# muzishen/RCDMs

Hardware: AMD Instinct MI355X
Metric: story-frames/sec (stage-2 UNet, 50-step DDIM, 512^2) (higher is better)
Workload: dtype f16; 1 GPU; PororoSV stage-2, 512x512, 50-step DDIM, CFG 2.0, batch=1 story x 5 frames per GPU, ctx 85x768, random-init 1276.9M-param UNet3D; stories_per_gpu=1, latent=64, ddim_steps=50, parallelism=story-replicas x1

## Files before the change

### rcdms_amd/csrc/igemm16.hip

```cpp
#include "common.h"
#include "igemm_args.h"
#include "pp_sync.h"
#include "igemm_epilogue.h"
#ifndef RCDM_I16_ABLATE
#define RCDM_I16_ABLATE 0
#endif

namespace {

template <int TAPS, bool SLAB>
__global__ __launch_bounds__(256, 2) void igemm16_kernel(const IgemmArgs p) {
  constexpr int BM = 160, BN = 160, FM = 5, FN = 5;
  constexpr int A_BYTES = BM * 128, STAGE = (BM + BN) * 128;
  constexpr int NP = BM / 8 / 4;
  extern __shared__ __attribute__((aligned(16))) char smem[];

  const int t = threadIdx.x, lane = t & 63;
  const int wave = __builtin_amdgcn_readfirstlane(t >> 6);
  const int wm = wave >> 1, wn = wave & 1;
  const int ks_begin = blockIdx.y * p.nk_per_split;
  const int nkl = min(p.nk, ks_begin + p.nk_per_split) - ks_begin;
  if (nkl <= 0) return;

  int cm0, cn0;
  {
    const int ntiles = p.tilesM * p.tilesN, lin = blockIdx.x;
    const int xcd = lin & 7, q = ntiles >> 3, r = ntiles & 7;
    const int tl = (xcd < r ? xcd * (q + 1) : r * (q + 1) + (xcd - r) * q) + (lin >> 3);
    constexpr int GM = 8;
    const int per_group = GM * p.tilesN;
    const int sg = tl / per_group, rem = tl - sg * per_group;
    const int gm = min(GM, p.tilesM - sg * GM);
    const int tn = rem / gm, tm = sg * GM + (rem - tn * gm);
    cm0 = tm * BM;
    cn0 = tn * BN;
  }

  f32x2 lx_pre = {1.f, 0.f};
  const bool lx_on = TAPS == 1 && !SLAB && p.lnx_stat != nullptr;
  LnxRow<1, kLnxMaxParts> lx_row0;
  if (lx_on && t < BM) lx_row0.load(p.lnx_stat, p.lnx_ld, cm0 + t, cm0 + t < p.M, p.lnx_parts, 0);

  const __amdgpu_buffer_rsrc_t rsrcA = __builtin_amdgcn_make_buffer_rsrc((void*)p.A, 0, 0x7FFFFFFF, 0x00020000);
  const __amdgpu_buffer_rsrc_t rsrcW = __builtin_amdgcn_make_buffer_rsrc((void*)p.W, 0, 0x7FFFFFFF, 0x00020000);
  const __amdgpu_buffer_rsrc_t rsrcA2 = __builtin_amdgcn_make_buffer_rsrc((void*)(TAPS == 9 ? p.A2 : p.A), 0, 0x7FFFFFFF, 0x00020000);
  constexpr unsigned OOB = 0x80000000u;
  const int Hv = p.Hi << p.up, Wv = p.Wi << p.up;
  const int lrow = lane >> 3, lch = lane & 7;

  unsigned a_off[NP], w_off[NP];
  int a_img[NP], a_iy[NP], a_ix[NP], a_c[NP], w_c[NP];
#pragma unroll
  for (int i = 0; i < NP; ++i) {
    const int row = (wave * NP + i) * 8 + lrow;
    const int m = cm0 + row;
    a_c[i] = (lch ^ ((row >> 1) & 7)) * 8;
    a_off[i] = OOB;
    a_img[i] = a_ix[i] = 0;
    a_iy[i] = -(1 << 20);
    if (TAPS == 1) {
      if (m < p.M) a_off[i] = (unsigned)m * (unsigned)p.lda * 2u;
    } else if (m < p.M) {
      const int hw = p.Ho * p.Wo;
      const int img = m / hw, rem = m - img * hw;
      const int oy = rem / p.Wo, ox = rem - oy * p.Wo;
      a_img[i] = img * p.Hi * p.Wi;
      a_iy[i] = oy * p.stride - p.pad;
      a_ix[i] = ox * p.stride - p.pad;
    }
    const int n = cn0 + row;
    w_c[i] = a_c[i];
    w_off[i] = n < p.N ? (unsigned)n * (unsigned)p.Ktot * 2u : OOB;
  }
  auto issue = [&](int g, int stage) __attribute__((always_inline)) {
    const int ks = ks_begin + g;
    int tap = 0, kci = ks;
    const bool s2 = TAPS == 9 && ks >= p.nk1;
    if (TAPS != 1) {
      kci = ks / 9;
      tap = ks - kci * 9;
      if (s2) {
        kci = ks - p.nk1;
        tap = 9;
      }
    }
    const int c0 = kci * BK;
    const int dy = s2 ? 1 : tap / 3, dx = s2 ? 1 : tap - dy * 3;
    const int cin = s2 ? p.Cin2 : p.Cin;
    const unsigned lda = (unsigned)(s2 ? p.lda2 : p.lda);
    char* sbase = smem + stage * STAGE;
#pragma unroll
    for (int i = 0; i < NP; ++i) {
      const int c = c0 + a_c[i];
      unsigned vo;
      if (TAPS == 1) {
        vo = (c < p.Cin && a_off[i] != OOB) ? a_off[i] + (unsigned)c * 2u : OOB;
      } else {
        const int iy = a_iy[i] + dy, ix = a_ix[i] + dx;
        const bool ok = (c < cin) && ((unsigned)iy < (unsigned)Hv) && ((unsigned)ix < (unsigned)Wv);
        const int sy = iy >> p.up, sx = ix >> p.up;
        const unsigned off = ((unsigned)(a_img[i] + sy * p.Wi + sx) * lda + (unsigned)c) * 2u;
        vo = ok ? off : OOB;
      }
      if (TAPS == 9 && s2)
        __builtin_amdgcn_raw_ptr_buffer_load_lds(
            rsrcA2, (__attribute__((address_space(3))) void*)(sbase + (wave * NP + i) * 1024), 16, vo, 0, 0, 0);
      else
        __builtin_amdgcn_raw_ptr_buffer_load_lds(
            rsrcA, (__attribute__((address_space(3))) void*)(sbase + (wave * NP + i) * 1024), 16, vo, 0, 0, 0);
    }
#if RCDM_I16_ABLATE & 16
    if (g > 0) return;
#endif
#pragma unroll
    for (int i = 0; i < NP; ++i) {
      const int c = c0 + w_c[i];
      const unsigned vo = (c < cin && w_off[i] != OOB)
                              ? w_off[i] + ((unsigned)tap * (unsigned)p.Cin + (unsigned)c) * 2u : OOB;
      __builtin_amdgcn_raw_ptr_buffer_load_lds(
          rsrcW, (__attribute__((address_space(3))) void*)(sbase + A_BYTES + (wave * NP + i) * 1024), 16, vo, 0, 0, 0);
    }
  };

  const int l15 = lane & 15, kg = lane >> 4;
  const int sw = (lane >> 1) & 7;
  const int koff0 = ((kg ^ sw) << 4), koff1 = (((4 + kg) ^ sw) << 4);
  const int rowA = (wm * (BM / 2) + l15) * 128, rowB = A_BYTES + (wn * (BN / 2) + l15) * 128;
  f32x4 acc[FN][FM];
#pragma unroll
  for (int i = 0; i < FN; ++i)
#pragma unroll
    for (int j = 0; j < FM; ++j) acc[i][j] = f32x4{0.f, 0.f, 0.f, 0.f};

  constexpr int kStg = BM * (2 * BN + 16);
  static_assert(lnx_table_bytes(BM, BN) <= 4096 && 4096 + kStg <= 2 * STAGE && kStg >= STAGE, "epilogue layout");
  const bool lx_low = lx_on && !(nkl & 1);
  float* const lx_tab = (float*)(smem + (lx_low ? 0 : kStg));
  char* const stg = smem + (lx_low ? 4096 : 0);
  issue(0, 0);
  if (lx_on && t < BM) {
    float r_ = 1.f, m_ = 0.f;
    lx_row0.finish(p.lnx_invC, p.lnx_eps, r_, m_);
    lx_pre = f32x2{r_, m_};
  }
  for (int g = 0; g < nkl; ++g) {
    wait_vm<0>();
    __builtin_amdgcn_s_barrier();
#if !(RCDM_I16_ABLATE & 8)
    if (g + 1 < nkl) issue(g + 1, (g + 1) & 1);
#endif
    const char* sb = smem + (g & 1) * STAGE;
#if RCDM_PRIO_LOADS
    __builtin_amdgcn_s_setprio(3);
#endif
#pragma unroll
    for (int kk = 0; kk < 2; ++kk) {
      const int koff = kk ? koff1 : koff0;
      f16x8 wf[FN], xf[FM];
#pragma unroll
      for (int i = 0; i < FN; ++i) wf[i] = *(const f16x8*)(sb + rowB + i * 2048 + koff);
#pragma unroll
      for (int j = 0; j < FM; ++j) xf[j] = *(const f16x8*)(sb + rowA + j * 2048 + koff);
#if RCDM_PRIO_LOADS
      __builtin_amdgcn_s_setprio(0);
#endif
#pragma unroll
      for (int i = 0; i < FN; ++i)
#pragma unroll
        for (int j = 0; j < FM; ++j) acc[i][j] = __builtin_amdgcn_mfma_f32_16x16x32_f16(wf[i], xf[j], acc[i][j], 0, 0, 0);
#if RCDM_PRIO_LOADS
      __builtin_amdgcn_s_setprio(3);
#endif
    }
  }
  if constexpr (TAPS == 1 && !SLAB)
    if (lx_on) lnx_write_tables<BM, BN>(p, lx_tab, cm0, cn0, t, lx_pre);
  wait_lgkm0();
  tick_barrier();
#if RCDM_I16_ABLATE & 1
  {
    float s = 0.f;
#pragma unroll
    for (int i = 0; i < FN; ++i)
#pragma unroll
      for (int j = 0; j < FM; ++j) s += acc[i][j][0] + acc[i][j][1] + acc[i][j][2] + acc[i][j][3];
    if (s == 1.2345678e33f) p.out[0] = (f16)s;
  }
#else
  if constexpr (SLAB) {
    if (p.slab16) {
      IgemmArgs q{};
      q.out = (f16*)p.partial + (size_t)blockIdx.y * p.M * p.N;
      q.M = p.M; q.N = p.N; q.ldc = p.N; q.epi = 0; q.out_scale = 1.0f; q.dup = 0;
      tile_epilogue<FM, FN, false, 256, BM, BN, false, false>(q, smem, acc, cm0, cn0, wm * (BM / 2), wn * (BN / 2), l15, kg, t, nullptr);
      return;
    }
  }
  tile_epilogue<FM, FN, SLAB, 256, BM, BN, false, TAPS == 1 && !SLAB>(p, stg, acc, cm0, cn0, wm * (BM / 2), wn * (BN / 2), l15, kg, t,
                                                                       lx_on ? lx_tab : nullptr);
#endif
}

constexpr int kLds16 = 2 * (160 + 160) * 128;

template <int TAPS>
int launch16(const IgemmArgs& a, hipStream_t stream) {
  static bool attr_set[64] = {};
  if (rcdm_first_on_device(attr_set)) {
    (void)hipFuncSetAttribute((const void*)igemm16_kernel<TAPS, false>, hipFuncAttributeMaxDynamicSharedMemorySize, kLds16);
    (void)hipFuncSetAttribute((const void*)igemm16_kernel<TAPS, true>, hipFuncAttributeMaxDynamicSharedMemorySize, kLds16);
  }
  dim3 grid(a.tilesM * a.tilesN, a.splits);
  if (a.splits > 1)
    hipLaunchKernelGGL((igemm16_kernel<TAPS, true>), grid, dim3(256), kLds16, stream, a);
  else
    hipLaunchKernelGGL((igemm16_kernel<TAPS, false>), grid, dim3(256), kLds16, stream, a);
  return rcdm_check_launch();
}

}

int rcdm_igemm16_launch(const IgemmArgs& a, int taps, hipStream_t stream) {
  if (taps == 1) return launch16<1>(a, stream);
  if (taps == 9) return launch16<9>(a, stream);
  return RCDM_EINVAL;
}
```

### rcdms_amd/csrc/wino.hip

```cpp
#include "common.h"
#include "igemm_args.h"
#include "pp_sync.h"
#include "igemm_epilogue.h"
#include <stdlib.h>

namespace {

struct WinoArgs {
  const f16* in;
  const f16* in2;
  const f16* U;
  const f16* W2;
  const float* bias;
  const float* rowvec;
  const f16* res;
  f16* out;
  f16* V;
  float* slab;
  int slab16;
  int n_img, H, W, th, tw, T, N, K, K2;
  int lda, lda2, ldc, ldr, ldt, rows_per_sample;
  int epi;
  float out_scale;
  int E, splits, nk, nk2, nkps, nkps2, tilesM, tilesN;
  const float* gn_stat;
  const float* gn_gamma;
  const float* gn_beta;
  int gn_cg, gn_G, gn_rps, gn_silu;
  float* go_partial;
  int go_G, go_cg, go_rps, go_splits;
};

__global__ __launch_bounds__(256) void wino_in_kernel(const WinoArgs p) {
  const int nch = p.K >> 2;
  const int idx = blockIdx.x * 256 + threadIdx.x;
  if (idx >= p.T * nch) return;
  const int t = idx / nch, c4 = idx - t * nch;
  const int tpi = p.th * p.tw;
  const int img = t / tpi, rem = t - img * tpi;
  const int ty = rem / p.tw, tx = rem - ty * p.tw;
  typedef unsigned u32x2_t __attribute__((ext_vector_type(2)));
  union H4 { u32x2_t v; f16 e[4]; f16x4 h; };
  const __amdgpu_buffer_rsrc_t rs = __builtin_amdgcn_make_buffer_rsrc((void*)p.in, 0, 0x7FFFFFFF, 0x00020000);
  const unsigned base = ((unsigned)(img * p.H * p.W) * (unsigned)p.lda + (unsigned)c4 * 4u) * 2u;
  H4 d[4][4];
  bool ok[4][4];
#pragma unroll
  for (int i = 0; i < 4; ++i)
#pragma unroll
    for (int j = 0; j < 4; ++j) {
      const int y = 2 * ty - 1 + i, x = 2 * tx - 1 + j;
      ok[i][j] = (unsigned)y < (unsigned)p.H && (unsigned)x < (unsigned)p.W;
      const unsigned off = ok[i][j] ? base + (unsigned)(y * p.W + x) * (unsigned)p.lda * 2u : 0x80000000u;
      d[i][j].v = __builtin_amdgcn_raw_buffer_load_b64(rs, off, 0, 0);
    }
  f32x4 sc = {1.f, 1.f, 1.f, 1.f}, sh = {0.f, 0.f, 0.f, 0.f};
  const bool gn = p.gn_stat != nullptr;
  if (gn) {
    const int s = (img * p.H * p.W) / p.gn_rps;
    const f32x4 ga = *(const f32x4*)(p.gn_gamma + c4 * 4), be = *(const f32x4*)(p.gn_beta + c4 * 4);
#pragma unroll
    for (int e = 0; e < 4; ++e) {
      const int g = (c4 * 4 + e) / p.gn_cg;
      const f32x2 mr = *(const f32x2*)(p.gn_stat + (size_t)(s * p.gn_G + g) * 2);
      sc[e] = mr.y * ga[e];
      sh[e] = __builtin_fmaf(-(mr.x * mr.y), ga[e], be[e]);
    }
  }
  float f[4][4][4];
#pragma unroll
  for (int i = 0; i < 4; ++i)
#pragma unroll
    for (int j = 0; j < 4; ++j)
#pragma unroll
      for (int e = 0; e < 4; ++e) {
        float v = (float)d[i][j].e[e];
        if (gn) {
          v = __builtin_fmaf(v, sc[e], sh[e]);
          if (p.gn_silu) v = silu_f(v);
          if (!ok[i][j]) v = 0.f;
        }
        f[i][j][e] = v;
      }
  float r[4][4][4];
#pragma unroll
  for (int j = 0; j < 4; ++j)
#pragma unroll
    for (int e = 0; e < 4; ++e) {
      r[0][j][e] = f[0][j][e] - f[2][j][e];
      r[1][j][e] = f[1][j][e] + f[2][j][e];
      r[2][j][e] = f[2][j][e] - f[1][j][e];
      r[3][j][e] = f[1][j][e] - f[3][j][e];
    }
  f16* vb = p.V + (size_t)t * p.K + c4 * 4;
  const size_t pstride = (size_t)p.T * p.K;
#pragma unroll
  for (int i = 0; i < 4; ++i) {
    H4 o[4];
#pragma unroll
    for (int e = 0; e < 4; ++e) {
      o[0].e[e] = (f16)(r[i][0][e] - r[i][2][e]);
      o[1].e[e] = (f16)(r[i][1][e] + r[i][2][e]);
      o[2].e[e] = (f16)(r[i][2][e] - r[i][1][e]);
      o[3].e[e] = (f16)(r[i][1][e] - r[i][3][e]);
    }
#pragma unroll
    for (int j = 0; j < 4; ++j) *(u32x2_t*)(vb + (size_t)(i * 4 + j) * pstride) = o[j].v;
  }
}

template <bool S16>
__global__ __launch_bounds__(256, 2) void wino_gemm_kernel(const WinoArgs p) {
  constexpr int BM = 160, BN = 160, FM = 5, FN = 5;
  constexpr int A_BYTES = BM * 128, STAGE = (BM + BN) * 128;
  constexpr int NP = BM / 8 / 4;
  extern __shared__ __attribute__((aligned(16))) char smem[];

  const int t = threadIdx.x, lane = t & 63;
  const int wave = __builtin_amdgcn_readfirstlane(t >> 6);
  const int wm = wave >> 1, wn = wave & 1;
  const int ntile = p.tilesM * p.tilesN, W = p.E * p.splits * ntile;
  const int n_extra = p.E - 16;
  int item;
  {
    const int lin = blockIdx.x, xcd = lin & 7, j = lin >> 3;
    const int WX = n_extra * p.splits * ntile, WM = W - WX;
    if (((WX | WM) & 7) == 0) {
      const int xq = WX >> 3, mq = WM >> 3;
      item = j < xq ? xcd * xq + j : WX + xcd * mq + (j - xq);
    } else {
      const int q = W >> 3, r = W & 7;
      item = (xcd < r ? xcd * (q + 1) : r * (q + 1) + (xcd - r) * q) + j;
    }
  }
  const int yes = item / ntile, tl = item - yes * ntile;
  const int ye = yes / p.splits, split = yes - ye * p.splits;
  const int entry = ye < n_extra ? 16 + ye : ye - n_extra;
  const bool extra = entry >= 16;
  const int nk = extra ? p.nk2 : p.nk, nkps = extra ? p.nkps2 : p.nkps;
  const int ks_begin = split * nkps;
  const int nkl = min(nk, ks_begin + nkps) - ks_begin;
  const int Kd = extra ? p.K2 : p.K;
  const size_t slab_off = ((size_t)entry * p.splits + split) * p.T * p.N;

  const int tn = tl / p.tilesM, tm = tl - tn * p.tilesM;
  const int cm0 = tm * BM, cn0 = tn * BN;
  const f16* Abase = extra ? p.in2 : p.V + (size_t)entry * p.T * p.K;
  const f16* Wbase = extra ? p.W2 : p.U + (size_t)entry * p.N * p.K;
  const __amdgpu_buffer_rsrc_t rsrcA = __builtin_amdgcn_make_buffer_rsrc((void*)Abase, 0, 0x7FFFFFFF, 0x00020000);
  const __amdgpu_buffer_rsrc_t rsrcW = __builtin_amdgcn_make_buffer_rsrc((void*)Wbase, 0, 0x7FFFFFFF, 0x00020000);
  constexpr unsigned OOB = 0x80000000u;
  const int lrow = lane >> 3, lch = lane & 7;

  unsigned a_off[NP], w_off[NP];
  int a_c[NP];
#pragma unroll
  for (int i = 0; i < NP; ++i) {
    const int row = (wave * NP + i) * 8 + lrow;
    const int m = cm0 + row;
    a_c[i] = (lch ^ ((row >> 1) & 7)) * 8;
    a_off[i] = OOB;
    if (m < p.T) {
      if (extra) {
        const int tpi = p.th * p.tw;
        const int img = m / tpi, rem = m - img * tpi;
        const int ty = rem / p.tw, tx = rem - ty * p.tw;
        const int ab = entry - 16;
        const int prow = img * p.H * p.W + (2 * ty + (ab >> 1)) * p.W + 2 * tx + (ab & 1);
        a_off[i] = (unsigned)prow * (unsigned)p.lda2 * 2u;
      } else {
        a_off[i] = (unsigned)m * (unsigned)p.K * 2u;
      }
    }
    const int n = cn0 + row;
    w_off[i] = n < p.N ? (unsigned)n * (unsigned)Kd * 2u : OOB;
  }
  auto issue = [&](int g, int stage) __attribute__((always_inline)) {
    const int c0 = (ks_begin + g) * BK;
    char* sbase = smem + stage * STAGE;
#pragma unroll
    for (int i = 0; i < NP; ++i) {
      const int c = c0 + a_c[i];
      const unsigned vo = (c < Kd && a_off[i] != OOB) ? a_off[i] + (unsigned)c * 2u : OOB;
      __builtin_amdgcn_raw_ptr_buffer_load_lds(
          rsrcA, (__attribute__((address_space(3))) void*)(sbase + (wave * NP + i) * 1024), 16, vo, 0, 0, 0);
    }
#pragma unroll
    for (int i = 0; i < NP; ++i) {
      const int c = c0 + a_c[i];
      const unsigned vo = (c < Kd && w_off[i] != OOB) ? w_off[i] + (unsigned)c * 2u : OOB;
      __builtin_amdgcn_raw_ptr_buffer_load_lds(
          rsrcW, (__attribute__((address_space(3))) void*)(sbase + A_BYTES + (wave * NP + i) * 1024), 16, vo, 0, 0, 0);
    }
  };

  const int l15 = lane & 15, kg = lane >> 4;
  const int sw = (lane >> 1) & 7;
  const int koff0 = ((kg ^ sw) << 4), koff1 = (((4 + kg) ^ sw) << 4);
  const int rowA = (wm * (BM / 2) + l15) * 128, rowB = A_BYTES + (wn * (BN / 2) + l15) * 128;
  f32x4 acc[FN][FM];
#pragma unroll
  for (int i = 0; i < FN; ++i)
#pragma unroll
    for (int j = 0; j < FM; ++j) acc[i][j] = f32x4{0.f, 0.f, 0.f, 0.f};

  if (nkl > 0) issue(0, 0);
  for (int g = 0; g < nkl; ++g) {
    wait_vm<0>();
    __builtin_amdgcn_s_barrier();
    if (g + 1 < nkl) issue(g + 1, (g + 1) & 1);
    const char* sb = smem + (g & 1) * STAGE;
    __builtin_amdgcn_s_setprio(3);
#pragma unroll
    for (int kk = 0; kk < 2; ++kk) {
      const int koff = kk ? koff1 : koff0;
      f16x8 wf[FN], xf[FM];
#pragma unroll
      for (int i = 0; i < FN; ++i) wf[i] = *(const f16x8*)(sb + rowB + i * 2048 + koff);
#pragma unroll
      for (int j = 0; j < FM; ++j) xf[j] = *(const f16x8*)(sb + rowA + j * 2048 + koff);
      __builtin_amdgcn_s_setprio(0);
#pragma unroll
      for (int i = 0; i < FN; ++i)
#pragma unroll
        for (int j = 0; j < FM; ++j) acc[i][j] = __builtin_amdgcn_mfma_f32_16x16x32_f16(wf[i], xf[j], acc[i][j], 0, 0, 0);
      __builtin_amdgcn_s_setprio(3);
    }
  }
  const int row0 = wm * (BM / 2), col0 = wn * (BN / 2);
  if constexpr (S16) {
    wait_lgkm0();
    tick_barrier();
    IgemmArgs q{};
    q.out = (f16*)p.slab + slab_off;
    q.M = p.T; q.N = p.N; q.ldc = p.N; q.epi = 0; q.out_scale = 1.0f; q.dup = 0;
    tile_epilogue<FM, FN, false, 256, BM, BN, false, false>(q, smem, acc, cm0, cn0, row0, col0, l15, kg, t, nullptr);
  } else {
    wait_lgkm0();
    tick_barrier();
    slab_store_staged<FM, FN, 256, BM, BN, 80>(p.slab + slab_off, p.N, p.T, p.N, smem, acc, cm0, cn0, row0, col0, l15, kg, t);
  }
}

template <bool S16>
__device__ __forceinline__ f32x4 slab_load4(const WinoArgs& p, size_t off) {
  if constexpr (S16) {
    union { uint2 u; f16 e[4]; } h;
    h.u = *(const uint2*)((const f16*)p.slab + off);
    return f32x4{(float)h.e[0], (float)h.e[1], (float)h.e[2], (float)h.e[3]};
  } else {
    return *(const f32x4*)(p.slab + off);
  }
}

template <int SP, bool S16>
__global__ __launch_bounds__(512) void wino_out_kernel(const WinoArgs p) {
  extern __shared__ __attribute__((aligned(16))) char smem[];
  const int nch = p.N >> 2;
  const int t = blockIdx.x;
  const int tpi = p.th * p.tw;
  const int img = t / tpi, rem = t - img * tpi;
  const int ty = rem / p.tw, tx = rem - ty * p.tw;
  const size_t splane = (size_t)p.T * p.N, eplane = (size_t)p.splits * splane;
  int prow[4];
#pragma unroll
  for (int ab = 0; ab < 4; ++ab) prow[ab] = img * p.H * p.W + (2 * ty + (ab >> 1)) * p.W + 2 * tx + (ab & 1);
  union H4 { uint2 u; f16 e[4]; };
  for (int cg4 = threadIdx.x; cg4 < nch; cg4 += blockDim.x) {
    const int n = cg4 * 4;
    const size_t src = (size_t)t * p.N + n;
    H4 rr[4];
#pragma unroll
    for (int ab = 0; ab < 4; ++ab) {
      rr[ab].u = make_uint2(0, 0);
      if (p.epi & RCDM_EPI_RESIDUAL) rr[ab].u = *(const uint2*)(p.res + (size_t)prow[ab] * p.ldr + n);
    }
    f32x4 m[16];
#pragma unroll
    for (int e = 0; e < 16; ++e) m[e] = slab_load4<S16>(p, src + e * eplane);
    if constexpr (SP == 2) {
      f32x4 m2[16];
#pragma unroll
      for (int e = 0; e < 16; ++e) m2[e] = slab_load4<S16>(p, src + e * eplane + splane);
#pragma unroll
      for (int e = 0; e < 16; ++e) m[e] += m2[e];
    } else if constexpr (SP == 0) {
      for (int s = 1; s < p.splits; ++s) {
        f32x4 m2[16];
#pragma unroll
        for (int e = 0; e < 16; ++e) m2[e] = slab_load4<S16>(p, src + e * eplane + s * splane);
#pragma unroll
        for (int e = 0; e < 16; ++e) m[e] += m2[e];
      }
    }
    f32x4 o[4];
    {
      f32x4 r0[4], r1[4];
#pragma unroll
      for (int j = 0; j < 4; ++j) {
        r0[j] = m[0 * 4 + j] + m[1 * 4 + j] + m[2 * 4 + j];
        r1[j] = m[1 * 4 + j] - m[2 * 4 + j] - m[3 * 4 + j];
      }
      o[0] = r0[0] + r0[1] + r0[2];
      o[1] = r0[1] - r0[2] - r0[3];
      o[2] = r1[0] + r1[1] + r1[2];
      o[3] = r1[1] - r1[2] - r1[3];
    }
    if (p.E > 16) {
      f32x4 x[4];
#pragma unroll
      for (int ab = 0; ab < 4; ++ab) x[ab] = slab_load4<S16>(p, src + (16 + ab) * eplane);
      for (int s = 1; s < p.splits; ++s) {
#pragma unroll
        for (int ab = 0; ab < 4; ++ab) x[ab] += slab_load4<S16>(p, src + (16 + ab) * eplane + s * splane);
      }
#pragma unroll
      for (int ab = 0; ab < 4; ++ab) o[ab] += x[ab];
    }
    f32x4 add = {0.f, 0.f, 0.f, 0.f};
    if (p.epi & RCDM_EPI_BIAS) add += *(const f32x4*)(p.bias + n);
    if (p.epi & RCDM_EPI_ROWVEC) add += *(const f32x4*)(p.rowvec + (size_t)(prow[0] / p.rows_per_sample) * p.ldt + n);
    f32x4 cs = {0.f, 0.f, 0.f, 0.f}, cq = cs;
#pragma unroll
    for (int ab = 0; ab < 4; ++ab) {
      H4 q;
#pragma unroll
      for (int e = 0; e < 4; ++e) {
        q.e[e] = (f16)((o[ab][e] + add[e] + (float)rr[ab].e[e]) * p.out_scale);
        const float f = (float)q.e[e];
        cs[e] += f;
        cq[e] += f * f;
      }
      *(uint2*)(p.out + (size_t)prow[ab] * p.ldc + n) = q.u;
    }
    if (p.go_partial) {
      *(f32x4*)(smem + (size_t)n * 4) = cs;
      *(f32x4*)(smem + (size_t)(p.N + n) * 4) = cq;
    }
  }
  if (p.go_partial) {
    __syncthreads();
    const int g = threadIdx.x;
    if (g < p.go_G) {
      const float* fs = (const float*)smem;
      float gs = 0.f, gq = 0.f;
      for (int c = g * p.go_cg; c < (g + 1) * p.go_cg; ++c) {
        gs += fs[c];
        gq += fs[p.N + c];
      }
      const float nn = 4.f * (float)p.go_cg;
      const float mean = gs / nn;
      float m2 = gq - gs * mean;
      if (m2 < 0.f) m2 = 0.f;
      const int s = prow[0] / p.go_rps;
      const int sp = t - s * p.go_splits;
      float* o = p.go_partial + (((size_t)s * p.go_G + g) * p.go_splits + sp) * 3;
      o[0] = nn;
      o[1] = mean;
      o[2] = m2;
    }
  }
}

__global__ __launch_bounds__(256) void wino_pack_kernel(const float* __restrict__ w, f16* __restrict__ U, int c_out, int c_in) {
  const size_t idx = (size_t)blockIdx.x * 256 + threadIdx.x;
  const size_t total = (size_t)c_out * c_in;
  if (idx >= total) return;
  const float* g = w + idx * 9;
  float gg[3][3];
#pragma unroll
  for (int i = 0; i < 3; ++i)
#pragma unroll
    for (int j = 0; j < 3; ++j) gg[i][j] = g[i * 3 + j];
  float r[4][3];
#pragma unroll
  for (int j = 0; j < 3; ++j) {
    r[0][j] = gg[0][j];
    r[1][j] = 0.5f * (gg[0][j] + gg[1][j] + gg[2][j]);
    r[2][j] = 0.5f * (gg[0][j] - gg[1][j] + gg[2][j]);
    r[3][j] = gg[2][j];
  }
#pragma unroll
  for (int i = 0; i < 4; ++i) {
    const float u0 = r[i][0], u1 = 0.5f * (r[i][0] + r[i][1] + r[i][2]), u2 = 0.5f * (r[i][0] - r[i][1] + r[i][2]), u3 = r[i][2];
    U[(size_t)(i * 4 + 0) * total + idx] = (f16)u0;
    U[(size_t)(i * 4 + 1) * total + idx] = (f16)u1;
    U[(size_t)(i * 4 + 2) * total + idx] = (f16)u2;
    U[(size_t)(i * 4 + 3) * total + idx] = (f16)u3;
  }
}

struct UpGatherArgs {
  const f16* P;
  const float* bias;
  f16* out;
  int ldp, ldc, n_img, H, W, C;
  int up;
};
__global__ __launch_bounds__(256) void upsample_gather_kernel(const UpGatherArgs p) {
  const int nch = p.C >> 3;
  const size_t total = ((size_t)p.n_img * p.H * p.W << (2 * p.up)) * nch;
  const size_t idx = (size_t)blockIdx.x * 256 + threadIdx.x;
  if (idx >= total) return;
  const int o = (int)(idx / nch), c8 = (int)(idx - (size_t)o * nch);
  const int W2 = p.W << p.up, H2 = p.H << p.up;
  const int img = o / (H2 * W2), rem = o - img * (H2 * W2);
  const int Y = rem / W2, X = rem - Y * W2;
  const __amdgpu_buffer_rsrc_t rs = __builtin_amdgcn_make_buffer_rsrc((void*)p.P, 0, 0x7FFFFFFF, 0x00020000);
  Pack16 v[9];
#pragma unroll
  for (int ky = 0; ky < 3; ++ky)
#pragma unroll
    for (int kx = 0; kx < 3; ++kx) {
      const int yy = Y + ky - 1, xx = X + kx - 1;
      const bool ok = (unsigned)yy < (unsigned)H2 && (unsigned)xx < (unsigned)W2;
      const unsigned row = (unsigned)(img * p.H * p.W + (yy >> p.up) * p.W + (xx >> p.up));
      const unsigned off = ok ? (row * (unsigned)p.ldp + (unsigned)((ky * 3 + kx) * p.C + c8 * 8)) * 2u : 0x80000000u;
      v[ky * 3 + kx].v = __builtin_amdgcn_raw_buffer_load_b128(rs, off, 0, 0);
    }
  float acc[8];
#pragma unroll
  for (int e = 0; e < 8; ++e) acc[e] = 0.f;
  if (p.bias) {
    const f32x4 b0 = *(const f32x4*)(p.bias + c8 * 8), b1 = *(const f32x4*)(p.bias + c8 * 8 + 4);
#pragma unroll
    for (int e = 0; e < 4; ++e) {
      acc[e] = b0[e];
      acc[4 + e] = b1[e];
    }
  }
#pragma unroll
  for (int k = 0; k < 9; ++k)
#pragma unroll
    for (int e = 0; e < 8; ++e) acc[e] += (float)v[k].e[e];
  Pack16 q;
#pragma unroll
  for (int e = 0; e < 8; ++e) q.e[e] = (f16)acc[e];
  *(uint4*)(p.out + (size_t)o * p.ldc + c8 * 8) = q.u;
}

int g_wino_cus = 0;
int wino_cus() {
  if (g_wino_cus <= 0) {
    int dev = 0, n = 0;
    if (hipGetDevice(&dev) == hipSuccess && hipDeviceGetAttribute(&n, hipDeviceAttributeMultiprocessorCount, dev) == hipSuccess && n > 0)
      g_wino_cus = n;
    else
      g_wino_cus = 256;
  }
  return g_wino_cus;
}

inline size_t align256(size_t v) { return (v + 255) & ~(size_t)255; }

int wino_plan(const rcdm_conv3x3_desc* d, WinoArgs& a) {
  if (!d) return RCDM_EINVAL;
  if (d->n_img <= 0 || d->h_in <= 0 || d->w_in <= 0 || d->c_in <= 0 || d->c_out <= 0) return RCDM_EINVAL;
  if (d->stride != 1 || d->upsample != 0 || d->pad_after_only || d->dup_rows) return RCDM_ESHAPE;
  if ((d->h_in & 1) || (d->w_in & 1)) return RCDM_ESHAPE;
  if ((d->c_in & 63) || (d->c_out & 7) || (d->c_in2 & 63)) return RCDM_ESHAPE;
  if ((d->lda & 7) || (d->ldc & 7) || (d->c_in2 && (d->lda2 & 7))) return RCDM_EINVAL;
  if (d->epilogue & ~(RCDM_EPI_BIAS | RCDM_EPI_ROWVEC | RCDM_EPI_RESIDUAL)) return RCDM_ESHAPE;
  if ((d->epilogue & RCDM_EPI_RESIDUAL) && (d->ldr & 7)) return RCDM_EINVAL;
  a = WinoArgs{};
  a.n_img = d->n_img; a.H = d->h_in; a.W = d->w_in;
  a.th = d->h_in / 2; a.tw = d->w_in / 2;
  a.T = d->n_img * a.th * a.tw;
  a.N = d->c_out; a.K = d->c_in; a.K2 = d->c_in2;
  a.lda = d->lda; a.lda2 = d->lda2; a.ldc = d->ldc; a.ldr = d->ldr; a.ldt = d->ldt;
  a.rows_per_sample = d->rows_per_sample > 0 ? d->rows_per_sample : 1;
  a.epi = d->epilogue;
  a.out_scale = d->out_scale == 0.f ? 1.f : d->out_scale;
  a.E = d->c_in2 ? 20 : 16;
  a.nk = d->c_in / BK; a.nk2 = d->c_in2 / BK;
  a.tilesM = (a.T + 159) / 160; a.tilesN = (a.N + 159) / 160;
  if ((size_t)a.T * a.K * 2 >= (1ull << 31)) return RCDM_ESHAPE;
  if ((size_t)d->n_img * d->h_in * d->w_in * d->lda * 2 >= (1ull << 31)) return RCDM_ESHAPE;
  if (d->c_in2 && (size_t)d->n_img * d->h_in * d->w_in * d->lda2 * 2 >= (1ull << 31)) return RCDM_ESHAPE;
  if ((size_t)a.N * (a.K > a.K2 ? a.K : a.K2) * 2 >= (1ull << 31)) return RCDM_ESHAPE;
  int splits = d->split_k;
  if (splits <= 0) {
    const int blocks = a.E * a.tilesM * a.tilesN;
    splits = wino_cus() / (blocks > 0 ? blocks : 1);
    if (splits > a.nk / 5) splits = a.nk / 5;
    if (splits > 8) splits = 8;
  }
  if (splits < 1) splits = 1;
  if (splits > a.nk) splits = a.nk;
  a.splits = splits;
  a.nkps = (a.nk + splits - 1) / splits;
  a.nkps2 = (a.nk2 + splits - 1) / splits;
  return RCDM_OK;
}
size_t wino_v_bytes(const WinoArgs& a) { return align256((size_t)16 * a.T * a.K * 2); }
size_t wino_slab_bytes(const WinoArgs& a) { return align256((size_t)a.E * a.splits * a.T * a.N * 4); }

int g_wino_slab16 = -1;
int wino_slab16() {
  if (g_wino_slab16 < 0) {
    const char* e = getenv("RCDM_WINO_SLAB16");
    g_wino_slab16 = e ? (atoi(e) != 0) : 1;
  }
  return g_wino_slab16;
}

}

extern "C" {

int rcdm_conv3x3_wino_supported(const rcdm_conv3x3_desc* d) {
  WinoArgs a;
  return wino_plan(d, a) == RCDM_OK ? 1 : 0;
}

size_t rcdm_conv3x3_wino_workspace_bytes(const rcdm_conv3x3_desc* d) {
  WinoArgs a;
  if (wino_plan(d, a) != RCDM_OK) return 0;
  return wino_v_bytes(a) + wino_slab_bytes(a);
}

int rcdm_conv3x3_wino_plan_query(const rcdm_conv3x3_desc* d, int32_t* out8) {
  WinoArgs a;
  const int rc = wino_plan(d, a);
  if (rc != RCDM_OK || !out8) return rc != RCDM_OK ? rc : RCDM_EINVAL;
  out8[0] = 11; out8[1] = 160; out8[2] = 160; out8[3] = a.tilesM; out8[4] = a.tilesN * a.E; out8[5] = a.splits; out8[6] = 2;
  out8[7] = a.nk;
  return RCDM_OK;
}

int rcdm_conv_taps_gather(const void* P, int32_t ldp, int32_t n_img, int32_t h, int32_t w, int32_t c_out, int32_t upsample,
                          const float* bias, void* out, int32_t ldc, void* stream) {
  if (!P || !out || n_img <= 0 || h <= 0 || w <= 0 || c_out <= 0 || (upsample != 0 && upsample != 1)) return RCDM_EINVAL;
  if ((c_out & 7) || (ldp & 7) || (ldc & 7) || ldp < 9 * c_out || ldc < c_out) return RCDM_EINVAL;
  if ((((uintptr_t)P | (uintptr_t)out | (uintptr_t)bias) & 15)) return RCDM_EINVAL;
  if ((size_t)n_img * h * w * ldp * 2 >= (1ull << 31)) return RCDM_ESHAPE;
  UpGatherArgs a{(const f16*)P, bias, (f16*)out, ldp, ldc, n_img, h, w, c_out, upsample};
  const size_t total = ((size_t)n_img * h * w << (2 * upsample)) * (c_out >> 3);
  hipLaunchKernelGGL(upsample_gather_kernel, dim3((unsigned)((total + 255) / 256)), dim3(256), 0, (hipStream_t)stream, a);
  return rcdm_check_launch();
}

int rcdm_upsample_taps_gather(const void* P, int32_t ldp, int32_t n_img, int32_t h, int32_t w, int32_t c_out, const float* bias,
                              void* out, int32_t ldc, void* stream) {
  return rcdm_conv_taps_gather(P, ldp, n_img, h, w, c_out, 1, bias, out, ldc, stream);
}

int rcdm_set_wino_slab_f16(int32_t on) {
  g_wino_slab16 = on < 0 ? -1 : (on ? 1 : 0);
  return RCDM_OK;
}

int rcdm_pack_conv3x3_wino(const float* w, int32_t c_out, int32_t c_in, void* dst, void* stream) {
  if (!w || !dst || c_out <= 0 || c_in <= 0) return RCDM_EINVAL;
  const size_t total = (size_t)c_out * c_in;
  hipLaunchKernelGGL(wino_pack_kernel, dim3((unsigned)((total + 255) / 256)), dim3(256), 0, (hipStream_t)stream, w, (f16*)dst, c_out, c_in);
  return rcdm_check_launch();
}

int rcdm_conv3x3_wino(const rcdm_conv3x3_desc* d, const rcdm_groupnorm_desc* gn, const float* gn_stat, const float* gn_gamma,
                      const float* gn_beta, const void* in, const void* in2, const void* U, const void* W2, const float* bias,
                      const float* rowvec, const void* residual, void* out, void* workspace, size_t workspace_bytes,
                      const rcdm_groupnorm_desc* gn_out, float* gn_out_partial, void* stream_) {
  WinoArgs a;
  const int rc = wino_plan(d, a);
  if (rc != RCDM_OK) return rc;
  if (!in || !U || !out || !workspace) return RCDM_EINVAL;
  if ((d->c_in2 != 0) != (in2 != nullptr) || (d->c_in2 != 0) != (W2 != nullptr)) return RCDM_EINVAL;
  if ((a.epi & RCDM_EPI_BIAS) && !bias) return RCDM_EINVAL;
  if ((a.epi & RCDM_EPI_ROWVEC) && (!rowvec || (d->ldt & 3))) return RCDM_EINVAL;
  if ((a.epi & RCDM_EPI_RESIDUAL) && !residual) return RCDM_EINVAL;
  if (workspace_bytes < wino_v_bytes(a) + wino_slab_bytes(a)) return RCDM_EWORKSPACE;
  if (((uintptr_t)in | (uintptr_t)out | (uintptr_t)U | (uintptr_t)workspace | (uintptr_t)in2 | (uintptr_t)W2 | (uintptr_t)residual |
       (uintptr_t)bias | (uintptr_t)rowvec) & 15)
    return RCDM_EINVAL;
  if (gn) {
    if (!gn_stat || !gn_gamma || !gn_beta) return RCDM_EINVAL;
    if (gn->C != d->c_in || gn->groups <= 0 || gn->C % gn->groups || gn->samples * gn->rows_per_sample != d->n_img * d->h_in * d->w_in ||
        gn->rows_per_sample % (d->h_in * d->w_in))
      return RCDM_ESHAPE;
    a.gn_stat = gn_stat; a.gn_gamma = gn_gamma; a.gn_beta = gn_beta;
    a.gn_G = gn->groups; a.gn_cg = gn->C / gn->groups; a.gn_rps = gn->rows_per_sample; a.gn_silu = gn->silu;
  }
  if (gn_out) {
    if (!gn_out_partial) return RCDM_EINVAL;
    if (gn_out->C != d->c_out || gn_out->groups <= 0 || gn_out->groups > 64 || gn_out->C % gn_out->groups ||
        gn_out->samples * gn_out->rows_per_sample != d->n_img * d->h_in * d->w_in || gn_out->rows_per_sample % (d->h_in * d->w_in) ||
        a.N * 8 > 64 * 1024)
      return RCDM_ESHAPE;
    a.go_partial = gn_out_partial;
    a.go_G = gn_out->groups; a.go_cg = gn_out->C / gn_out->groups; a.go_rps = gn_out->rows_per_sample;
    a.go_splits = gn_out->rows_per_sample / 4;
  }
  a.in = (const f16*)in; a.in2 = (const f16*)in2; a.U = (const f16*)U; a.W2 = (const f16*)W2;
  a.bias = bias; a.rowvec = rowvec; a.res = (const f16*)residual; a.out = (f16*)out;
  a.V = (f16*)workspace;
  a.slab16 = wino_slab16();
  a.slab = (float*)((char*)workspace + wino_v_bytes(a));
  hipStream_t stream = (hipStream_t)stream_;
  {
    const size_t items = (size_t)a.T * (a.K >> 2);
    hipLaunchKernelGGL(wino_in_kernel, dim3((unsigned)((items + 255) / 256)), dim3(256), 0, stream, a);
  }
  {
    constexpr int kLds = 2 * (160 + 160) * 128;
    static bool attr_set[64] = {};
    if (rcdm_first_on_device(attr_set)) {
      (void)hipFuncSetAttribute((const void*)wino_gemm_kernel<false>, hipFuncAttributeMaxDynamicSharedMemorySize, kLds);
      (void)hipFuncSetAttribute((const void*)wino_gemm_kernel<true>, hipFuncAttributeMaxDynamicSharedMemorySize, kLds);
    }
    if (a.slab16) hipLaunchKernelGGL(wino_gemm_kernel<true>, dim3(a.tilesM * a.tilesN * a.E * a.splits), dim3(256), kLds, stream, a);
    else hipLaunchKernelGGL(wino_gemm_kernel<false>, dim3(a.tilesM * a.tilesN * a.E * a.splits), dim3(256), kLds, stream, a);
  }
  {
    int threads = ((a.N >> 2) + 63) / 64 * 64;
    if (threads > 512) threads = 512;
    const size_t lds = a.go_partial ? (size_t)a.N * 8 : 0;
    const dim3 grid((unsigned)a.T);
    if (a.slab16) {
      if (a.splits == 1) hipLaunchKernelGGL((wino_out_kernel<1, true>), grid, dim3(threads), lds, stream, a);
      else if (a.splits == 2) hipLaunchKernelGGL((wino_out_kernel<2, true>), grid, dim3(threads), lds, stream, a);
      else hipLaunchKernelGGL((wino_out_kernel<0, true>), grid, dim3(threads), lds, stream, a);
    } else {
      if (a.splits == 1) hipLaunchKernelGGL((wino_out_kernel<1, false>), grid, dim3(threads), lds, stream, a);
      else if (a.splits == 2) hipLaunchKernelGGL((wino_out_kernel<2, false>), grid, dim3(threads), lds, stream, a);
      else hipLaunchKernelGGL((wino_out_kernel<0, false>), grid, dim3(threads), lds, stream, a);
    }
  }
  return rcdm_check_launch();
}

}
```

Measured before the change: 6.032 story-frames/s.

## Interleave next-stage global loads and LDS fragment reads with MFMAs in igemm16

Restructures the igemm16 main loop so the prefetch of the next K-stage is split into per-row pieces and issued between MFMA groups, rather than as one burst at the top of the iteration. For the 3x3 and slab variants it also double-buffers the second-half LDS fragment reads behind the first half's MFMAs, with sched_barriers pinning the order. The last iteration is peeled so the prefetch branch leaves the loop body. The Winograd kernel is moved onto the shared helper but keeps burst mode, so it should behave as before. The risks are higher register pressure from the extra fragment buffers, which matters under launch_bounds(256,2), and a rigid schedule that may block the compiler's own reordering.

```diff
diff --git a/rcdms_amd/csrc/i16_loop.h b/rcdms_amd/csrc/i16_loop.h
--- /dev/null
+++ b/rcdms_amd/csrc/i16_loop.h
@@ -0,0 +1,109 @@
+#pragma once
+#include "common.h"
+#include "igemm_args.h"
+
+#ifndef RCDM_I16_PLACE
+#define RCDM_I16_PLACE 0
+#endif
+
+constexpr int kI16Place[7][5] = {
+    {0, 1, 2, 3, 4},
+    {0, 0, 1, 1, 2},
+    {1, 3, 5, 7, 9},
+    {5, 6, 7, 8, 9},
+    {-1, -1, -1, -1, -1},
+    {0, 0, 0, 0, 0},
+    {-2, -2, -2, -2, -2},
+};
+
+template <bool MORE, class Issue>
+__device__ __forceinline__ void i16_kstep(const char* sb, int rowA, int rowB, int koff0, int koff1, f32x4 (&acc)[5][5],
+                                          Issue&& issue) {
+  constexpr int F = 5;
+  f16x8 wf[F], xf[F], xg[F];
+  if constexpr (MORE) {
+#pragma unroll
+    for (int q = 0; q < F; ++q)
+      if (kI16Place[RCDM_I16_PLACE][q] == -2) { issue(q, 0); issue(q, 1); }
+  }
+#if RCDM_PRIO_LOADS
+  __builtin_amdgcn_s_setprio(3);
+#endif
+#pragma unroll
+  for (int j = 0; j < F; ++j) xf[j] = *(const f16x8*)(sb + rowA + j * 2048 + koff0);
+#pragma unroll
+  for (int i = 0; i < F; ++i) wf[i] = *(const f16x8*)(sb + rowB + i * 2048 + koff0);
+#if RCDM_PRIO_LOADS
+  __builtin_amdgcn_s_setprio(0);
+#endif
+  if constexpr (MORE && RCDM_I16_PLACE >= 4) {
+#pragma unroll
+    for (int q = 0; q < F; ++q)
+      if (kI16Place[RCDM_I16_PLACE][q] == -1) { issue(q, 0); issue(q, 1); }
+    __builtin_amdgcn_sched_barrier(0);
+  }
+#pragma unroll
+  for (int i = 0; i < F; ++i) {
+#pragma unroll
+    for (int j = 0; j < F; ++j) acc[i][j] = __builtin_amdgcn_mfma_f32_16x16x32_f16(wf[i], xf[j], acc[i][j], 0, 0, 0);
+    wf[i] = *(const f16x8*)(sb + rowB + i * 2048 + koff1);
+    xg[i] = *(const f16x8*)(sb + rowA + i * 2048 + koff1);
+    if constexpr (MORE) {
+#pragma unroll
+      for (int q = 0; q < F; ++q)
+        if (kI16Place[RCDM_I16_PLACE][q] == i) { issue(q, 0); issue(q, 1); }
+    }
+    __builtin_amdgcn_sched_barrier(0);
+  }
+#pragma unroll
+  for (int i = 0; i < F; ++i) {
+#pragma unroll
+    for (int j = 0; j < F; ++j) acc[i][j] = __builtin_amdgcn_mfma_f32_16x16x32_f16(wf[i], xg[j], acc[i][j], 0, 0, 0);
+    if constexpr (MORE) {
+#pragma unroll
+      for (int q = 0; q < F; ++q)
+        if (kI16Place[RCDM_I16_PLACE][q] == F + i) { issue(q, 0); issue(q, 1); }
+      if constexpr (RCDM_I16_PLACE >= 2) __builtin_amdgcn_sched_barrier(0);
+    }
+  }
+}
+
+template <bool MORE, class Issue>
+__device__ __forceinline__ void i16_kstep_burst(const char* sb, int rowA, int rowB, int koff0, int koff1, f32x4 (&acc)[5][5],
+                                                Issue&& issue) {
+  constexpr int F = 5;
+  if constexpr (MORE) {
+#pragma unroll
+    for (int part = 0; part < 2; ++part)
+#pragma unroll
+      for (int q = 0; q < F; ++q) issue(q, part);
+  }
+#if RCDM_PRIO_LOADS
+  __builtin_amdgcn_s_setprio(3);
+#endif
+#pragma unroll
+  for (int kk = 0; kk < 2; ++kk) {
+    const int koff = kk ? koff1 : koff0;
+    f16x8 wf[F], xf[F];
+#pragma unroll
+    for (int i = 0; i < F; ++i) wf[i] = *(const f16x8*)(sb + rowB + i * 2048 + koff);
+#pragma unroll
+    for (int j = 0; j < F; ++j) xf[j] = *(const f16x8*)(sb + rowA + j * 2048 + koff);
+#if RCDM_PRIO_LOADS
+    __builtin_amdgcn_s_setprio(0);
+#endif
+#pragma unroll
+    for (int i = 0; i < F; ++i)
+#pragma unroll
+      for (int j = 0; j < F; ++j) acc[i][j] = __builtin_amdgcn_mfma_f32_16x16x32_f16(wf[i], xf[j], acc[i][j], 0, 0, 0);
+#if RCDM_PRIO_LOADS
+    __builtin_amdgcn_s_setprio(3);
+#endif
+  }
+}
+
+template <bool MORE, bool INTERLEAVE, class Issue>
+__device__ __forceinline__ void i16_step(const char* sb, int rowA, int rowB, int koff0, int koff1, f32x4 (&acc)[5][5], Issue&& issue) {
+  if constexpr (INTERLEAVE) i16_kstep<MORE>(sb, rowA, rowB, koff0, koff1, acc, issue);
+  else i16_kstep_burst<MORE>(sb, rowA, rowB, koff0, koff1, acc, issue);
+}
diff --git a/rcdms_amd/csrc/igemm16.hip b/rcdms_amd/csrc/igemm16.hip
--- a/rcdms_amd/csrc/igemm16.hip
+++ b/rcdms_amd/csrc/igemm16.hip
@@ -2,11 +2,19 @@
 #include "igemm_args.h"
 #include "pp_sync.h"
 #include "igemm_epilogue.h"
+#include "i16_loop.h"
 #ifndef RCDM_I16_ABLATE
 #define RCDM_I16_ABLATE 0
 #endif
 
 namespace {
+
+struct Step {
+  int c0, tap, dy, dx, cin;
+  unsigned lda;
+  bool s2, wts;
+  char* sbase;
+};
 
 template <int TAPS, bool SLAB>
 __global__ __launch_bounds__(256, 2) void igemm16_kernel(const IgemmArgs p) {
@@ -72,53 +80,53 @@
     w_c[i] = a_c[i];
     w_off[i] = n < p.N ? (unsigned)n * (unsigned)p.Ktot * 2u : OOB;
   }
-  auto issue = [&](int g, int stage) __attribute__((always_inline)) {
+  auto step_of = [&](int g) __attribute__((always_inline)) {
     const int ks = ks_begin + g;
-    int tap = 0, kci = ks;
-    const bool s2 = TAPS == 9 && ks >= p.nk1;
+    Step s;
+    s.tap = 0;
+    int kci = ks;
+    s.s2 = TAPS == 9 && ks >= p.nk1;
     if (TAPS != 1) {
       kci = ks / 9;
-      tap = ks - kci * 9;
-      if (s2) {
+      s.tap = ks - kci * 9;
+      if (s.s2) {
         kci = ks - p.nk1;
-        tap = 9;
+        s.tap = 9;
       }
     }
-    const int c0 = kci * BK;
-    const int dy = s2 ? 1 : tap / 3, dx = s2 ? 1 : tap - dy * 3;
-    const int cin = s2 ? p.Cin2 : p.Cin;
-    const unsigned lda = (unsigned)(s2 ? p.lda2 : p.lda);
-    char* sbase = smem + stage * STAGE;
-#pragma unroll
-    for (int i = 0; i < NP; ++i) {
-      const int c = c0 + a_c[i];
+    s.c0 = kci * BK;
+    s.dy = s.s2 ? 1 : s.tap / 3;
+    s.dx = s.s2 ? 1 : s.tap - s.dy * 3;
+    s.cin = s.s2 ? p.Cin2 : p.Cin;
+    s.lda = (unsigned)(s.s2 ? p.lda2 : p.lda);
+    s.wts = true;
+#if RCDM_I16_ABLATE & 16
+    s.wts = g == 0;
+#endif
+    s.sbase = smem + (g & 1) * STAGE;
+    return s;
+  };
+  auto issue = [&](const Step& s, int i, int part) __attribute__((always_inline)) {
+    if (part == 0) {
+      const int c = s.c0 + a_c[i];
       unsigned vo;
       if (TAPS == 1) {
-        vo = (c < p.Cin && a_off[i] != OOB) ? a_off[i] + (unsigned)c * 2u : OOB;
+        vo = ((c < p.Cin) & (a_off[i] != OOB)) ? a_off[i] + (unsigned)c * 2u : OOB;
       } else {
-        const int iy = a_iy[i] + dy, ix = a_ix[i] + dx;
-        const bool ok = (c < cin) && ((unsigned)iy < (unsigned)Hv) && ((unsigned)ix < (unsigned)Wv);
+        const int iy = a_iy[i] + s.dy, ix = a_ix[i] + s.dx;
+        const bool ok = (c < s.cin) & ((unsigned)iy < (unsigned)Hv) & ((unsigned)ix < (unsigned)Wv);
         const int sy = iy >> p.up, sx = ix >> p.up;
-        const unsigned off = ((unsigned)(a_img[i] + sy * p.Wi + sx) * lda + (unsigned)c) * 2u;
+        const unsigned off = ((unsigned)(a_img[i] + sy * p.Wi + sx) * s.lda + (unsigned)c) * 2u;
         vo = ok ? off : OOB;
       }
-      if (TAPS == 9 && s2)
-        __builtin_amdgcn_raw_ptr_buffer_load_lds(
-            rsrcA2, (__attribute__((address_space(3))) void*)(sbase + (wave * NP + i) * 1024), 16, vo, 0, 0, 0);
-      else
-        __builtin_amdgcn_raw_ptr_buffer_load_lds(
-            rsrcA, (__attribute__((address_space(3))) void*)(sbase + (wave * NP + i) * 1024), 16, vo, 0, 0, 0);
-    }
-#if RCDM_I16_ABLATE & 16
-    if (g > 0) return;
-#endif
-#pragma unroll
-    for (int i = 0; i < NP; ++i) {
-      const int c = c0 + w_c[i];
-      const unsigned vo = (c < cin && w_off[i] != OOB)
-                              ? w_off[i] + ((unsigned)tap * (unsigned)p.Cin + (unsigned)c) * 2u : OOB;
       __builtin_amdgcn_raw_ptr_buffer_load_lds(
-          rsrcW, (__attribute__((address_space(3))) void*)(sbase + A_BYTES + (wave * NP + i) * 1024), 16, vo, 0, 0, 0);
+          TAPS == 9 && s.s2 ? rsrcA2 : rsrcA, (__attribute__((address_space(3))) void*)(s.sbase + (wave * NP + i) * 1024), 16, vo, 0, 0, 0);
+    } else if (s.wts) {
+      const int c = s.c0 + w_c[i];
+      const unsigned vo = ((c < s.cin) & (w_off[i] != OOB))
+                              ? w_off[i] + ((unsigned)s.tap * (unsigned)p.Cin + (unsigned)c) * 2u : OOB;
+      __builtin_amdgcn_raw_ptr_buffer_load_lds(
+          rsrcW, (__attribute__((address_space(3))) void*)(s.sbase + A_BYTES + (wave * NP + i) * 1024), 16, vo, 0, 0, 0);
     }
   };
 
@@ -137,41 +145,34 @@
   const bool lx_low = lx_on && !(nkl & 1);
   float* const lx_tab = (float*)(smem + (lx_low ? 0 : kStg));
   char* const stg = smem + (lx_low ? 4096 : 0);
-  issue(0, 0);
+  {
+    const Step s0 = step_of(0);
+#pragma unroll
+    for (int part = 0; part < 2; ++part)
+#pragma unroll
+      for (int i = 0; i < NP; ++i) issue(s0, i, part);
+  }
   if (lx_on && t < BM) {
     float r_ = 1.f, m_ = 0.f;
     lx_row0.finish(p.lnx_invC, p.lnx_eps, r_, m_);
     lx_pre = f32x2{r_, m_};
   }
-  for (int g = 0; g < nkl; ++g) {
+  static_assert(NP == FM && NP == FN, "i16_kstep issues one pixel and one weight piece per MFMA row");
+  constexpr bool kInterleave = TAPS == 9 || SLAB;
+  int g = 0;
+#if !(RCDM_I16_ABLATE & 8)
+  for (; g + 1 < nkl; ++g) {
     wait_vm<0>();
     __builtin_amdgcn_s_barrier();
-#if !(RCDM_I16_ABLATE & 8)
-    if (g + 1 < nkl) issue(g + 1, (g + 1) & 1);
-#endif
-    const char* sb = smem + (g & 1) * STAGE;
-#if RCDM_PRIO_LOADS
-    __builtin_amdgcn_s_setprio(3);
-#endif
-#pragma unroll
-    for (int kk = 0; kk < 2; ++kk) {
-      const int koff = kk ? koff1 : koff0;
-      f16x8 wf[FN], xf[FM];
-#pragma unroll
-      for (int i = 0; i < FN; ++i) wf[i] = *(const f16x8*)(sb + rowB + i * 2048 + koff);
-#pragma unroll
-      for (int j = 0; j < FM; ++j) xf[j] = *(const f16x8*)(sb + rowA + j * 2048 + koff);
-#if RCDM_PRIO_LOADS
-      __builtin_amdgcn_s_setprio(0);
-#endif
-#pragma unroll
-      for (int i = 0; i < FN; ++i)
-#pragma unroll
-        for (int j = 0; j < FM; ++j) acc[i][j] = __builtin_amdgcn_mfma_f32_16x16x32_f16(wf[i], xf[j], acc[i][j], 0, 0, 0);
-#if RCDM_PRIO_LOADS
-      __builtin_amdgcn_s_setprio(3);
-#endif
-    }
+    const Step sn = step_of(g + 1);
+    i16_step<true, kInterleave>(smem + (g & 1) * STAGE, rowA, rowB, koff0, koff1, acc,
+                                [&](int i, int part) __attribute__((always_inline)) { issue(sn, i, part); });
+  }
+#endif
+  for (; g < nkl; ++g) {
+    wait_vm<0>();
+    __builtin_amdgcn_s_barrier();
+    i16_step<false, kInterleave>(smem + (g & 1) * STAGE, rowA, rowB, koff0, koff1, acc, [](int, int) {});
   }
   if constexpr (TAPS == 1 && !SLAB)
     if (lx_on) lnx_write_tables<BM, BN>(p, lx_tab, cm0, cn0, t, lx_pre);
diff --git a/rcdms_amd/csrc/wino.hip b/rcdms_amd/csrc/wino.hip
--- a/rcdms_amd/csrc/wino.hip
+++ b/rcdms_amd/csrc/wino.hip
@@ -2,6 +2,7 @@
 #include "igemm_args.h"
 #include "pp_sync.h"
 #include "igemm_epilogue.h"
+#include "i16_loop.h"
 #include <stdlib.h>
 
 namespace {
@@ -175,19 +176,14 @@
     const int n = cn0 + row;
     w_off[i] = n < p.N ? (unsigned)n * (unsigned)Kd * 2u : OOB;
   }
-  auto issue = [&](int g, int stage) __attribute__((always_inline)) {
-    const int c0 = (ks_begin + g) * BK;
-    char* sbase = smem + stage * STAGE;
-#pragma unroll
-    for (int i = 0; i < NP; ++i) {
-      const int c = c0 + a_c[i];
+  auto issue = [&](int g, int i, int part) __attribute__((always_inline)) {
+    const int c = (ks_begin + g) * BK + a_c[i];
+    char* sbase = smem + (g & 1) * STAGE;
+    if (part == 0) {
       const unsigned vo = (c < Kd && a_off[i] != OOB) ? a_off[i] + (unsigned)c * 2u : OOB;
       __builtin_amdgcn_raw_ptr_buffer_load_lds(
           rsrcA, (__attribute__((address_space(3))) void*)(sbase + (wave * NP + i) * 1024), 16, vo, 0, 0, 0);
-    }
-#pragma unroll
-    for (int i = 0; i < NP; ++i) {
-      const int c = c0 + a_c[i];
+    } else {
       const unsigned vo = (c < Kd && w_off[i] != OOB) ? w_off[i] + (unsigned)c * 2u : OOB;
       __builtin_amdgcn_raw_ptr_buffer_load_lds(
           rsrcW, (__attribute__((address_space(3))) void*)(sbase + A_BYTES + (wave * NP + i) * 1024), 16, vo, 0, 0, 0);
@@ -204,28 +200,25 @@
 #pragma unroll
     for (int j = 0; j < FM; ++j) acc[i][j] = f32x4{0.f, 0.f, 0.f, 0.f};
 
-  if (nkl > 0) issue(0, 0);
-  for (int g = 0; g < nkl; ++g) {
+  static_assert(NP == FM && NP == FN, "i16_kstep issues one tile and one weight piece per MFMA row");
+  if (nkl > 0) {
+#pragma unroll
+    for (int part = 0; part < 2; ++part)
+#pragma unroll
+      for (int i = 0; i < NP; ++i) issue(0, i, part);
+  }
+  constexpr bool kInterleave = false;
+  int g = 0;
+  for (; g + 1 < nkl; ++g) {
     wait_vm<0>();
     __builtin_amdgcn_s_barrier();
-    if (g + 1 < nkl) issue(g + 1, (g + 1) & 1);
-    const char* sb = smem + (g & 1) * STAGE;
-    __builtin_amdgcn_s_setprio(3);
-#pragma unroll
-    for (int kk = 0; kk < 2; ++kk) {
-      const int koff = kk ? koff1 : koff0;
-      f16x8 wf[FN], xf[FM];
-#pragma unroll
-      for (int i = 0; i < FN; ++i) wf[i] = *(const f16x8*)(sb + rowB + i * 2048 + koff);
-#pragma unroll
-      for (int j = 0; j < FM; ++j) xf[j] = *(const f16x8*)(sb + rowA + j * 2048 + koff);
-      __builtin_amdgcn_s_setprio(0);
-#pragma unroll
-      for (int i = 0; i < FN; ++i)
-#pragma unroll
-        for (int j = 0; j < FM; ++j) acc[i][j] = __builtin_amdgcn_mfma_f32_16x16x32_f16(wf[i], xf[j], acc[i][j], 0, 0, 0);
-      __builtin_amdgcn_s_setprio(3);
-    }
+    i16_step<true, kInterleave>(smem + (g & 1) * STAGE, rowA, rowB, koff0, koff1, acc,
+                                [&](int i, int part) __attribute__((always_inline)) { issue(g + 1, i, part); });
+  }
+  if (g < nkl) {
+    wait_vm<0>();
+    __builtin_amdgcn_s_barrier();
+    i16_step<false, kInterleave>(smem + (g & 1) * STAGE, rowA, rowB, koff0, koff1, acc, [](int, int) {});
   }
   const int row0 = wm * (BM / 2), col0 = wn * (BN / 2);
   if constexpr (S16) {
```

Result: no change. 6.069 story-frames/s, median of 6 (+0.6%).
